# Rudrabha/Wav2Lip

Hardware: AMD Instinct MI355X
Metric: face-frames/sec (96x96, mel T=16) (higher is better)
Workload: dtype f32

## Files before the change

### include/w2l_hip.h

```cpp
#ifndef W2L_HIP_H
#define W2L_HIP_H

#include <stddef.h>
#include <stdint.h>

#ifdef __cplusplus
extern "C" {
#endif

#define W2L_OK 0
#define W2L_ERR_ARG (-1)
#define W2L_ERR_HIP (-2)
#define W2L_ERR_NOMEM (-3)

#define W2L_ACT_NONE 0
#define W2L_ACT_RELU 1
#define W2L_ACT_SIGMOID 2
#define W2L_ACT_LEAKY 3

#define W2L_PREC_F32 0
#define W2L_PREC_BF16 1

const char* w2l_last_error(void);
int w2l_abi_version(void);
// ... 201 lines not shown
                     float* dgamma, float* dbeta, float* dz, int dz_cs, float* g_out, int g_cs);
int w2l_act_bwd(void* stream, long long rows, int C, const float* dy, int dy_cs, const float* y, int y_cs, int act,
                const float* scale, float* dz, int dz_cs, float* g_out, int g_cs);
int w2l_add_rows(void* stream, long long rows, int C, const float* a, int a_cs, const float* b, int b_cs, float* out,
                 int out_cs);
int w2l_col_sum(void* stream, long long rows, int C, const float* x, int x_cs, float* out);

int w2l_l1_mean(void* stream, long long n, const float* a, const float* b, float* loss_out);
int w2l_l1_bwd(void* stream, long long n, const float* a, const float* b, const float* gout, float* da);
int w2l_cosine_bce_bwd(void* stream, int N, int C, const float* a, const float* v, const float* y, const float* gout,
                       float* da, float* dv);
int w2l_l2norm_bwd(void* stream, int N, int C, const float* x, int x_cs, const float* dy, float* dx, int dx_cs);
int w2l_bce_bwd(void* stream, int N, const float* p, const float* y, const float* gout, float* dp);

int w2l_shifted_pdist(void* stream, int T, int C, int vshift, const float* f1, const float* f2, float* out);

typedef struct w2l_adam_tensor {
    float* param;
    const float* grad;
    float* exp_avg;
    float* exp_avg_sq;
    long long n;
} w2l_adam_tensor;
typedef struct w2l_adam w2l_adam_t;
int w2l_adam_create(int ntensors, const long long* sizes_host, w2l_adam_t** out);
int w2l_adam_destroy(w2l_adam_t* h);
int w2l_adam_step(w2l_adam_t* h, void* stream, const w2l_adam_tensor* tensors_host, float lr, float beta1, float beta2,
                  float eps, float weight_decay, int step);


typedef struct w2l_plan w2l_plan_t;
int w2l_plan_create(w2l_plan_t** out);
int w2l_plan_destroy(w2l_plan_t* p);
int w2l_plan_add_conv(w2l_plan_t* p, const w2l_conv_t* c, int N, int H, int W, const float* x, int x_cs,
                      float* y, int y_cs, const float* res, int res_cs);
int w2l_plan_add_convb(w2l_plan_t* p, const w2l_convb_t* c, int N, int H, int W, const void* x, int x_cs, void* y, int y_cs,
                       const void* res, int res_cs, const float* scale, const float* shift);
int w2l_plan_add_convb_head(w2l_plan_t* p, const w2l_convb_t* c, int N, int H, int W, const void* x, int x_cs, uint8_t* frames,
                            float* y32, int y32_cs, const float* scale, const float* shift);
int w2l_plan_copy_item(w2l_plan_t* dst, const w2l_plan_t* src, int index);
int w2l_plan_run(const w2l_plan_t* p, void* stream);
int w2l_plan_size(const w2l_plan_t* p);
int w2l_plan_autotune(w2l_plan_t* p, void* stream, int reps);
int w2l_plan_get_config(const w2l_plan_t* p, int index, int* tile, int* ksplit);
int w2l_plan_set_config(w2l_plan_t* p, int index, int tile, int ksplit);
int w2l_plan_executed_flops(const w2l_plan_t* p, long long* flops_out, int* config_out);
int w2l_conv_num_igemm_tiles(void);
int w2l_flops_begin(void);
long long w2l_flops_end(long long* by_family);
int w2l_clock_probe(void* stream, int spin_us, unsigned long long* out2_dev);
int w2l_conv_config_family(int id);
int w2l_conv_exclude_families(int mask);
int w2l_igemm_block_order(int order, int order_r, int tiles_m, int tiles_n, int nphase, int* out);
int w2l_plan_profile(const w2l_plan_t* p, void* stream, int reps, float* ms_out);

#define W2L_TUNE_KEY_INTS 17
int w2l_tune_key_ints(void);
int w2l_tune_set(const int* key, int tile, int ksplit);
int w2l_tune_entry_applicable(const int* key, int tile);
int w2l_tune_clear(void);
int w2l_tune_count(void);
int w2l_tune_export(int* out, int cap_entries);

#ifdef __cplusplus
}
#endif
#endif
```

### wav2lip_amd/_lib.py

```python
import ctypes as C
import os

_HERE = os.path.dirname(os.path.abspath(__file__))
LIB_PATH = os.environ.get("W2L_HIP_LIB") or os.path.join(_HERE, "lib", "libw2l_hip.so")

ACT_NONE, ACT_RELU, ACT_SIGMOID, ACT_LEAKY = 0, 1, 2, 3
PREC_F32, PREC_BF16 = 0, 1


class ConvGeom(C.Structure):
    _fields_ = [(n, C.c_int) for n in
                ("transposed", "cin", "cout", "kh", "kw", "sh", "sw", "ph", "pw", "oph", "opw", "act")]


class AdamTensor(C.Structure):
    _fields_ = [("param", C.c_void_p), ("grad", C.c_void_p), ("exp_avg", C.c_void_p), ("exp_avg_sq", C.c_void_p),
                ("n", C.c_longlong)]


class WgradInfo(C.Structure):
    _fields_ = [(n, C.c_int) for n in ("family", "cfg", "ksplit", "chunk", "K", "kstep", "reduce_blocks")]


class WgradBf16Info(C.Structure):
# ... 82 lines not shown
                                     C.POINTER(C.c_int)]),
    "w2l_convb_forward_actbwd": (_i, [_vp, _vp, _i, _i, _i, _vp, _i, _vp, _i, _vp, _i, _vp, _i, _i, _vp, C.POINTER(C.c_int)]),
    "w2l_convb_set_tile": (_i, [_vp, _i]),
    "w2l_convb_num_tiles": (_i, []),
    "w2l_convb_resolve": (_i, [_vp, _i, _i, _i, _i, C.POINTER(C.c_int), C.POINTER(C.c_int), C.POINTER(C.c_int)]),
    "w2l_conv_wgrad_bf16": (_i, [C.POINTER(ConvGeom), _vp, _i, _i, _i, _vp, _i, _vp, _i, _vp]),
    "w2l_conv_wgrad_bf16_resolve": (_i, [C.POINTER(ConvGeom), _i, _i, _i, _i, _i, C.POINTER(WgradBf16Info)]),
    "w2l_bn_train_stats_bf16": (_i, [_vp, _ll, _i, _i, _vp, _i, _vp, _vp, _f, _f, _vp, _vp, _vp, _vp, _vp, _vp]),
    "w2l_affine_act_bf16": (_i, [_vp, _ll, _i, _vp, _i, _vp, _vp, _vp, _i, _i, _vp, _i]),
    "w2l_bn_train_bwd_bf16": (_i, [_vp, _ll, _i, _i, _vp, _i, _vp, _i, _vp, _i, _i, _vp, _vp, _vp, _vp, _vp, _vp, _vp, _i, _vp, _i]),
    "w2l_bn_train_bwd_apply_bf16": (_i, [_vp, _ll, _i, _vp, _i, _vp, _i, _vp, _i, _i, _vp, _vp, _vp, _vp, _vp, _vp, _vp, _i, _vp, _i]),
    "w2l_act_bwd_bf16": (_i, [_vp, _ll, _i, _vp, _i, _vp, _i, _i, _vp, _vp, _i, _vp, _i]),
    "w2l_add_rows_bf16": (_i, [_vp, _ll, _i, _vp, _i, _vp, _i, _vp, _i]),
    "w2l_col_sum_bf16": (_i, [_vp, _ll, _i, _vp, _i, _vp]),
    "w2l_thin1x1_forward_bf16": (_i, [_vp, _ll, _i, _i, _vp, _i, _vp, _vp, _i, _vp, _i]),
    "w2l_thin1x1_dgrad_bf16": (_i, [_vp, _ll, _i, _i, _vp, _i, _vp, _vp, _i, _vp, _i]),
    "w2l_thin1x1_wgrad_bf16": (_i, [_vp, _ll, _i, _i, _vp, _i, _vp, _i, _vp, _vp]),
    "w2l_thin1x1_wgrad_blocks": (_i, [_ll]),
    "w2l_nchw_to_nhwc_bf16": (_i, [_vp, _i, _i, _i, _i, _vp, _vp, _i, _i]),
    "w2l_nhwc_bf16_to_nchw": (_i, [_vp, _i, _i, _i, _i, _vp, _i, _vp]),
    "w2l_bn_train_stats": (_i, [_vp, _ll, _i, _vp, _i, _vp, _vp, _f, _f, _vp, _vp, _vp, _vp, _vp, _vp]),
    "w2l_affine_act": (_i, [_vp, _ll, _i, _vp, _i, _vp, _vp, _vp, _i, _i, _vp, _i]),
    "w2l_bn_train_bwd": (_i, [_vp, _ll, _i, _vp, _i, _vp, _i, _vp, _i, _i, _vp, _vp, _vp, _vp, _vp, _vp, _i, _vp, _i]),
    "w2l_act_bwd": (_i, [_vp, _ll, _i, _vp, _i, _vp, _i, _i, _vp, _vp, _i, _vp, _i]),
    "w2l_add_rows": (_i, [_vp, _ll, _i, _vp, _i, _vp, _i, _vp, _i]),
    "w2l_col_sum": (_i, [_vp, _ll, _i, _vp, _i, _vp]),
    "w2l_l1_mean": (_i, [_vp, _ll, _vp, _vp, _vp]),
    "w2l_l1_bwd": (_i, [_vp, _ll, _vp, _vp, _vp, _vp]),
    "w2l_cosine_bce_bwd": (_i, [_vp, _i, _i, _vp, _vp, _vp, _vp, _vp, _vp]),
    "w2l_l2norm_bwd": (_i, [_vp, _i, _i, _vp, _i, _vp, _vp, _i]),
    "w2l_bce_bwd": (_i, [_vp, _i, _vp, _vp, _vp, _vp]),
    "w2l_shifted_pdist": (_i, [_vp, _i, _i, _i, _vp, _vp, _vp]),
    "w2l_adam_create": (_i, [_i, C.POINTER(_ll), C.POINTER(_vp)]),
    "w2l_adam_destroy": (_i, [_vp]),
    "w2l_adam_step": (_i, [_vp, _vp, C.POINTER(AdamTensor), _f, _f, _f, _f, _f, _i]),
    "w2l_plan_create": (_i, [C.POINTER(_vp)]),
    "w2l_plan_destroy": (_i, [_vp]),
    "w2l_plan_add_conv": (_i, [_vp, _vp, _i, _i, _i, _vp, _i, _vp, _i, _vp, _i]),
    "w2l_plan_add_convb": (_i, [_vp, _vp, _i, _i, _i, _vp, _i, _vp, _i, _vp, _i, _vp, _vp]),
    "w2l_plan_add_convb_head": (_i, [_vp, _vp, _i, _i, _i, _vp, _i, _vp, _vp, _i, _vp, _vp]),
    "w2l_plan_copy_item": (_i, [_vp, _vp, _i]),
    "w2l_plan_run": (_i, [_vp, _vp]),
    "w2l_plan_size": (_i, [_vp]),
    "w2l_plan_autotune": (_i, [_vp, _vp, _i]),
    "w2l_plan_get_config": (_i, [_vp, _i, C.POINTER(_i), C.POINTER(_i)]),
    "w2l_plan_set_config": (_i, [_vp, _i, _i, _i]),
    "w2l_plan_profile": (_i, [_vp, _vp, _i, _vp]),
    "w2l_plan_executed_flops": (_i, [_vp, C.POINTER(_ll), C.POINTER(_i)]),
    "w2l_conv_num_igemm_tiles": (_i, []),
    "w2l_flops_begin": (_i, []),
    "w2l_flops_end": (_ll, [C.POINTER(_ll)]),
    "w2l_clock_probe": (C.c_int, [C.c_void_p, C.c_int, C.c_void_p]),
    "w2l_igemm_block_order": (C.c_int, [C.c_int, C.c_int, C.c_int, C.c_int, C.c_int, C.c_void_p]),
    "w2l_conv_config_family": (_i, [_i]),
    "w2l_conv_exclude_families": (_i, [_i]),
    "w2l_tune_key_ints": (_i, []),
    "w2l_tune_set": (_i, [C.POINTER(_i), _i, _i]),
    "w2l_tune_entry_applicable": (_i, [C.POINTER(_i), _i]),
    "w2l_tune_clear": (_i, []),
    "w2l_tune_count": (_i, []),
    "w2l_tune_export": (_i, [C.POINTER(_i), _i]),
}

_lib = None

TUNE_TABLE_PATH = os.path.join(_HERE, "tune_table.json")
EXACT = os.environ.get("W2L_EXACT", "0") == "1"
EXACT_TABLE_PATH = os.path.join(_HERE, "tune_table_exact.json")
FAMILY_NAMES = ("igemm", "wino", "wino2", "tp2", "wino4", "split", "wino2s", "tp2s", "stem7s", "k3s")
SPLIT_FAMILIES = frozenset(FAMILY_NAMES.index(n) for n in ("split", "wino2s", "tp2s", "stem7s", "k3s"))
FAMILY_WINO4, FAMILY_SPLIT, FAMILY_WINO2S, FAMILY_TP2S, FAMILY_STEM7S, FAMILY_K3S = (
    FAMILY_NAMES.index(n) for n in ("wino4", "split", "wino2s", "tp2s", "stem7s", "k3s"))


def config_ids(lib, family):
    f = FAMILY_NAMES.index(family)
    return [i for i in range(lib.w2l_conv_num_tiles()) if lib.w2l_conv_config_family(i) == f]


NO_SPLIT = os.environ.get("W2L_SPLIT", "1") == "0"
NOSPLIT_TABLE_PATH = os.path.join(_HERE, "tune_table_nosplit.json")


def load_tune_table(lib, path=None):
    import json
    if path is None and NO_SPLIT and not EXACT and not os.environ.get("W2L_TUNE_TABLE"):
        return load_tune_table(lib, TUNE_TABLE_PATH) + load_tune_table(lib, NOSPLIT_TABLE_PATH)
    path = path or os.environ.get("W2L_TUNE_TABLE") or (EXACT_TABLE_PATH if EXACT else TUNE_TABLE_PATH)
    if path == "0" or not os.path.exists(path):
        return 0
    with open(path) as fh:
        doc = json.load(fh)
    nk = lib.w2l_tune_key_ints()
    if doc.get("key_ints") != nk or doc.get("num_configs", 0) > lib.w2l_conv_num_tiles():
        raise RuntimeError("tune table %s was written for another library build (key_ints %s / configs %s)"
                           % (path, doc.get("key_ints"), doc.get("num_configs")))
    n = 0
    for e in doc["entries"]:
        key = (C.c_int * nk)(*e[:nk])
        check_rc = lib.w2l_tune_set(key, int(e[nk]), int(e[nk + 1]))
        if check_rc != 0:
            raise RuntimeError("tune table %s: bad entry %s" % (path, e))
        n += 1
    return n


# ... 58 lines not shown
```

### wav2lip_amd/csrc/conv_wino4.hip

```cpp
#include "w2l_common.h"
#include "w2l_pk.h"

namespace w2l {

typedef float f32x16 __attribute__((ext_vector_type(16)));
typedef unsigned int u32x4 __attribute__((ext_vector_type(4)));

__device__ __forceinline__ f32x2 pk2_mul4(f32x2 a) {
    f32x2 d;
    asm("v_pk_mul_f32 %0, %1, 4.0 op_sel_hi:[1,0]" : "=v"(d) : "v"(a));
    return d;
}

template <int BLK>
__device__ __forceinline__ void w4_at3(f32x2 m0, f32x2 m1, f32x2 m2, f32x2& o0, f32x2& o1, f32x2& o2, f32x2& o3) {
    if (BLK == 0) {
        const f32x2 sm = pk2_add(m1, m2);
        o1 = pk2_sub(m1, m2);
        o0 = pk2_add(m0, sm);
        o2 = sm;
        o3 = o1;
    } else {
        const f32x2 sm = pk2_add(m0, m1);
        const f32x2 df = pk2_sub(m0, m1);
// ... 9 lines not shown
    f32x2 R[4][3];
#pragma unroll
    for (int jl = 0; jl < 3; ++jl) {
        const f32x2 m0 = {acc[0 + jl][r], acc[0 + jl][r + 1]};
        const f32x2 m1 = {acc[3 + jl][r], acc[3 + jl][r + 1]};
        const f32x2 m2 = {acc[6 + jl][r], acc[6 + jl][r + 1]};
        w4_at3<PI>(m0, m1, m2, R[0][jl], R[1][jl], R[2][jl], R[3][jl]);
    }
    f32x2 P1[4];
#pragma unroll
    for (int oa = 0; oa < 4; ++oa) {
        f32x2 P[4];
        if (PI == 0 && oa == 3) {
#pragma unroll
            for (int ob = 0; ob < 4; ++ob) P[ob] = P1[ob];
        } else {
            w4_at3<PJ>(R[oa][0], R[oa][1], R[oa][2], P[0], P[1], P[2], P[3]);
        }
        if (oa == 1) {
#pragma unroll
            for (int ob = 0; ob < 4; ++ob) P1[ob] = P[ob];
        }
        float* yo = y + (oa * 4) * LDY;
#pragma unroll
        for (int ob = 0; ob < 4; ++ob) {
            yo[ob * LDY] = P[ob].x;
            yo[ob * LDY + tstride] = P[ob].y;
        }
    }
}

#ifndef W4_DBG
#define W4_DBG 0
#endif
#ifdef W4_TRACE
__device__ unsigned long long w4_trace_buf[256 * 16 * 8];
__device__ unsigned long long w4_trace_rt[256 * 16 * 2];
#define W4_STAMP(k)                                                                                              \
    do {                                                                                                         \
        if (threadIdx.x == 0 && trace_item < 16) {                                                               \
            w4_trace_buf[(blockIdx.x * 16 + trace_item) * 8 + (k)] = __builtin_readcyclecounter();              \
            if ((k) == 0 || (k) == 7)                                                                            \
                w4_trace_rt[(blockIdx.x * 16 + trace_item) * 2 + ((k) ? 1 : 0)] = __builtin_amdgcn_s_memrealtime(); \
        }                                                                                                        \
    } while (0)
#else
#define W4_STAMP(k)
#endif

constexpr unsigned kW4Oob = 0x80000000u;
constexpr int kW4BT = 32;
constexpr int kW4BC = 64;
constexpr int kW4KS = 8;
constexpr int kW4LDK = kW4KS + 4;
constexpr int kW4VPOS = kW4BT * kW4LDK;
constexpr int kW4VBUF = 36 * kW4VPOS;
constexpr int kW4NRAW = 3;
constexpr int kW4RAW4 = 512 * kW4NRAW;
constexpr int kW4PS = 186;
constexpr int kW4QS = 4 * kW4PS;
static_assert(2 * kW4QS <= kW4RAW4 && kW4PS % 8 == 2 && kW4QS % 16 == 8, "raw plane geometry");
constexpr int kW4LDY = kW4BC + 4;
constexpr int kW4LdsFloats = 2 * kW4VBUF + 2 * kW4RAW4 * 4;
constexpr int kW4LdsBytes = kW4LdsFloats * 4 + 2 * kW4BT * 4;
static_assert(4 * kW4BT * 4 * kW4LDY <= kW4LdsFloats, "one round of the four partial staging tiles must fit");
static_assert(kW4LdsBytes <= 160 * 1024, "LDS budget");

struct Wino4KArgs {
    const float* x;
    float* y;
    const float* res;
    const float* u;
    const float* scale;
    const float* shift;
    int N, H, W, cin, x_cs;
    int cout, y_cs, res_cs;
    int TH, TW;
    int bh, bw, ni;
    int nby, nbx, ngi;
    int RH, RW, R4;
    int pitch, istride;
    float inv_rw, inv_rh;
    int nks;
    int tiles_n;
    long long total;
    int act;
};

__global__ __launch_bounds__(512, 2) void conv_wino4_f32_kernel(const Wino4KArgs a) {
    extern __shared__ __attribute__((aligned(16))) char smem[];
    float* Vs = reinterpret_cast<float*>(smem);
    float* Rs = Vs + 2 * kW4VBUF;
    int* s_opix = reinterpret_cast<int*>(Rs + 2 * kW4RAW4 * 4);
    int* s_oflag = s_opix + kW4BT;

    const __amdgpu_buffer_rsrc_t rx = __builtin_amdgcn_make_buffer_rsrc(
        const_cast<float*>(a.x), 0, (int)((((long long)a.N * a.H * a.W - 1) * a.x_cs + a.cin) * 4), 0x00020000);

    const unsigned total = (unsigned)a.total;
    const unsigned per = (total + 7u) / 8u;
    const unsigned xcd = blockIdx.x & 7u, gw = gridDim.x >> 3;
#ifdef W4_TRACE
    int trace_item = -1;
#endif
    for (unsigned jw = blockIdx.x >> 3; jw < per; jw += gw) {
    const unsigned bid = xcd * per + jw;
    if (bid >= total) break;
#ifdef W4_TRACE
    ++trace_item;
#endif
    W4_STAMP(0);
    int t = threadIdx.x;
    asm volatile("" : "+v"(t));
    const int lane = t & 63;
    const int wave = __builtin_amdgcn_readfirstlane(t >> 6);
    const int wn = wave & 1;
    const int pb = wave >> 1;
    const int PI = pb >> 1, PJ = pb & 1;
    const int tile_n = (int)(bid % (unsigned)a.tiles_n);
    unsigned mb = bid / (unsigned)a.tiles_n;
    const int bx_i = (int)(mb % (unsigned)a.nbx);
    mb /= (unsigned)a.nbx;
    const int by_i = (int)(mb % (unsigned)a.nby);
    const int gi = (int)(mb / (unsigned)a.nby);
    const int n0 = tile_n * kW4BC;
    const int bhw = a.bh * a.bw;

    if (t < kW4BT) {
        const int il = t / bhw, r = t - il * bhw;
        const int tyl = r / a.bw, txl = r - tyl * a.bw;
        const int n = gi * a.ni + il, ty = by_i * a.bh + tyl, tx = bx_i * a.bw + txl;
        int o = -1, f = 0;
        if (il < a.ni && n < a.N && ty < a.TH && tx < a.TW) {
            o = (n * a.H + 4 * ty) * a.W + 4 * tx;
#pragma unroll
            for (int k = 0; k < 4; ++k) f |= ((4 * ty + k < a.H) ? (1 << k) : 0) | ((4 * tx + k < a.W) ? (16 << k) : 0);
        }
        s_opix[t] = o;
        s_oflag[t] = f;
    }

    unsigned goff[kW4NRAW];
    int rst[kW4NRAW];
#pragma unroll
    for (int k = 0; k < kW4NRAW; ++k) {
        const int e = t + 512 * k;
        const int q = (e >> 3) & 1, pix = (e >> 4) * 8 + (e & 7);
        unsigned off = kW4Oob;
        int st = -1;
        if (pix < a.R4) {
            const int p2 = (int)(((float)pix + 0.5f) * a.inv_rw);
            const int rxx = pix - p2 * a.RW;
            const int il = (int)(((float)p2 + 0.5f) * a.inv_rh);
            const int ry = p2 - il * a.RH;
            st = (q * kW4QS + (rxx & 3) * kW4PS + il * a.istride + ry * a.pitch + (rxx >> 2)) * 16;
            const int n = gi * a.ni + il;
            const int iy = 4 * by_i * a.bh - 1 + ry, ix = 4 * bx_i * a.bw - 1 + rxx;
            if (n < a.N && (unsigned)iy < (unsigned)a.H && (unsigned)ix < (unsigned)a.W)
                off = ((unsigned)((n * a.H + iy) * a.W + ix) * (unsigned)a.x_cs + (unsigned)(q * 4)) * 4u;
        }
        goff[k] = off;
        rst[k] = st;
    }
    f32x4 rawreg[kW4NRAW];
    auto raw_gload = [&](int step) {
        const unsigned soff = (unsigned)(step * kW4KS * 4);
#pragma unroll
        for (int k = 0; k < kW4NRAW; ++k)
            rawreg[k] = __builtin_bit_cast(f32x4, __builtin_amdgcn_raw_buffer_load_b128(rx, (int)goff[k], (int)soff, 0));
    };
    auto raw_store = [&](int buf) {
        char* dst = reinterpret_cast<char*>(Rs) + buf * (kW4RAW4 * 16);
#pragma unroll
        for (int k = 0; k < kW4NRAW; ++k)
            if (rst[k] >= 0) *reinterpret_cast<f32x4*>(dst + rst[k]) = rawreg[k];
    };

    const bool tf_wave = wave < 6;
    const int q = lane & 1;
    int ra, rb, rc, rd;
    float ca, cb, cc;
    switch (wave) {
        case 0: ra = 0; ca = 0.f; rb = 0; cb = 4.f; rc = 2; cc = -5.f; rd = 4; break;
        case 1: ra = 1; ca = -4.f; rb = 2; cb = -4.f; rc = 3; cc = 1.f; rd = 4; break;
        case 2: ra = 1; ca = 4.f; rb = 2; cb = -4.f; rc = 3; cc = -1.f; rd = 4; break;
        case 3: ra = 1; ca = -2.f; rb = 2; cb = -1.f; rc = 3; cc = 2.f; rd = 4; break;
        case 4: ra = 1; ca = 2.f; rb = 2; cb = -1.f; rc = 3; cc = -2.f; rd = 4; break;
        default: ra = 1; ca = 0.f; rb = 1; cb = 4.f; rc = 3; cc = -5.f; rd = 5; break;
    }
    int tf_base;
    {
        const int tl = lane >> 1;
        const int il = tl / bhw, r = tl - il * bhw;
        const int tyl = r / a.bw, txl = r - tyl * a.bw;
        const int ilc = il < a.ni ? il : 0;
        tf_base = (q * kW4QS + ilc * a.istride + 4 * tyl * a.pitch + txl) * 16;
    }
    const int rp = a.pitch * 16;
    const int o_a = tf_base + ra * rp, o_b = tf_base + rb * rp, o_c = tf_base + rc * rp, o_d = tf_base + rd * rp;
    float* const vwr = Vs + ((wave < 6 ? wave : 0) * 6) * kW4VPOS + (lane >> 1) * kW4LDK + q * 4;
    f32x4 rr[6];
    auto tf_rows = [&](int buf, int c0) {
        const char* src = reinterpret_cast<const char*>(Rs) + buf * (kW4RAW4 * 16);
#pragma unroll
        for (int c = c0; c < c0 + 1; ++c) {
            const int co = ((c & 3) * kW4PS + (c >> 2)) * 16;
            const f32x4 va = *reinterpret_cast<const f32x4*>(src + o_a + co), vb = *reinterpret_cast<const f32x4*>(src + o_b + co);
            const f32x4 vc = *reinterpret_cast<const f32x4*>(src + o_c + co), vd = *reinterpret_cast<const f32x4*>(src + o_d + co);
#pragma unroll
            for (int e = 0; e < 4; ++e) rr[c][e] = fmaf(ca, va[e], fmaf(cb, vb[e], fmaf(cc, vc[e], vd[e])));
        }
    };
    auto tf_cols_store = [&](int buf) {
        float* dst = vwr + buf * kW4VBUF;
        f32x4 v0, v1, v2, v3, v4, v5;
#pragma unroll
        for (int e = 0; e < 4; ++e) {
            const float p = fmaf(-4.f, rr[2][e], rr[4][e]);
            const float qq = fmaf(4.f, rr[1][e], -rr[3][e]);
            const float p2 = rr[4][e] - rr[2][e];
            const float q2 = 2.f * (rr[3][e] - rr[1][e]);
            v0[e] = fmaf(4.f, rr[0][e], fmaf(-5.f, rr[2][e], rr[4][e]));
            v1[e] = p - qq;
            v2[e] = p + qq;
            v3[e] = p2 + q2;
            v4[e] = p2 - q2;
            v5[e] = fmaf(4.f, rr[1][e], fmaf(-5.f, rr[3][e], rr[5][e]));
        }
        *reinterpret_cast<f32x4*>(dst + 0 * kW4VPOS) = v0;
        *reinterpret_cast<f32x4*>(dst + 1 * kW4VPOS) = v1;
        *reinterpret_cast<f32x4*>(dst + 2 * kW4VPOS) = v2;
        *reinterpret_cast<f32x4*>(dst + 3 * kW4VPOS) = v3;
        *reinterpret_cast<f32x4*>(dst + 4 * kW4VPOS) = v4;
        *reinterpret_cast<f32x4*>(dst + 5 * kW4VPOS) = v5;
    };

    const int nb = (n0 >> 5) + wn;
    const int F = a.nks * 36;
    const __amdgpu_buffer_rsrc_t ru = __builtin_amdgcn_make_buffer_rsrc(
        const_cast<float*>(a.u + (long long)nb * F * 256), 0, F * 1024, 0x00020000);
    const unsigned bl_lane = (unsigned)(lane * 16);
    const int pos0 = 18 * PI + 3 * PJ;
    const unsigned bl_pb = (unsigned)pos0 * 1024u;
    auto bload = [&](int kc, int s) {
        const unsigned soff = (unsigned)kc * 36864u + bl_pb + (unsigned)(6 * (s / 3) + (s % 3)) * 1024u;
        return __builtin_bit_cast(f32x4, __builtin_amdgcn_raw_buffer_load_b128(ru, (int)bl_lane, (int)soff, 0));
    };
    constexpr int RING = 3;
    f32x4 bq[RING];

    f32x16 acc[9];
#pragma unroll
    for (int s = 0; s < 9; ++s)
#pragma unroll
        for (int r = 0; r < 16; ++r) acc[s][r] = 0.f;

    const int nsteps = a.cin / kW4KS;
    raw_gload(0);
#pragma unroll
    for (int i = 0; i < RING; ++i) bq[i] = bload(0, i);
    raw_store(0);
    raw_gload(1);
    __syncthreads();
    W4_STAMP(1);
    if (tf_wave) {
#pragma unroll
        for (int c = 0; c < 6; ++c) tf_rows(0, c);
        tf_cols_store(0);
    }
    raw_store(1);
    __syncthreads();
    W4_STAMP(2);

    const float* Abase = Vs + pos0 * kW4VPOS + (lane & 31) * kW4LDK + (lane >> 5) * 4;
    for (int step = 0; step < nsteps; ++step) {
        const int buf = step & 1;
        const float* Ab = Abase + buf * kW4VBUF;
        f32x4 af = *reinterpret_cast<const f32x4*>(Ab);
#pragma unroll
        for (int s = 0; s < 9; ++s) {
            const f32x4 ac = af;
            if (s < 8) af = *reinterpret_cast<const f32x4*>(Ab + (6 * ((s + 1) / 3) + ((s + 1) % 3)) * kW4VPOS);
            const f32x4 bc = bq[s % RING];
#if !(W4_DBG & 8)
            bq[s % RING] = (s < 9 - RING) ? bload(step, s + RING) : bload(step + 1, s + RING - 9);
#endif
            if (s == 0) {
                if (!(W4_DBG & 4)) raw_gload(step + 2);
            } else if (s >= 1 && s <= 6) {
                if (!(W4_DBG & 2) && tf_wave) tf_rows(buf ^ 1, s - 1);
            } else if (s == 7) {
                if (!(W4_DBG & 2) && tf_wave) tf_cols_store(buf ^ 1);
            } else if (s == 8) {
                if (!(W4_DBG & 4)) raw_store(buf);
            }
            __builtin_amdgcn_sched_barrier(0);
#if W4_DBG & 1
            asm volatile("" : "+v"(acc[s]) : "v"(ac), "v"(bc));
#else
#pragma unroll
            for (int e = 0; e < 4; ++e) acc[s] = __builtin_amdgcn_mfma_f32_32x32x2f32(ac[e], bc[e], acc[s], 0, 0, 0);
#endif
            __builtin_amdgcn_sched_barrier(0);
        }
        __syncthreads();
    }

    W4_STAMP(3);
    float* Ys = Vs;
    const long long npix = (long long)a.N * a.H * a.W;
    const __amdgpu_buffer_rsrc_t ry =
        __builtin_amdgcn_make_buffer_rsrc(a.y, 0, (int)(((npix - 1) * a.y_cs + a.cout) * 4), 0x00020000);
    const __amdgpu_buffer_rsrc_t rres = __builtin_amdgcn_make_buffer_rsrc(
        const_cast<float*>(a.res ? a.res : a.y), 0, a.res ? (int)(((npix - 1) * a.res_cs + a.cout) * 4) : 0, 0x00020000);
    constexpr int CG = kW4BC / 4;
    const int c4 = t % CG;
    const int ch = n0 + c4 * 4;
    const f32x4 sc = *reinterpret_cast<const f32x4*>(a.scale + ch);
    const f32x4 sh = *reinterpret_cast<const f32x4*>(a.shift + ch);
    const float neg_slope = a.act == W2L_ACT_RELU ? 0.f : (a.act == W2L_ACT_LEAKY ? 0.01f : 1.f);
    constexpr int kPart = 8 * 16 * kW4LDY;
    constexpr int NIT = 8 * 16 * CG / 512;
    auto out_pix = [&](int round, int i) {
        const int id = i * 512 + t;
        const int pxl = id / CG;
        const int tile = 8 * round + (pxl >> 4), oa = (pxl >> 2) & 3, ob = pxl & 3;
        const int opix = s_opix[tile];
        const int fl = s_oflag[tile];
        const bool ok = (opix >= 0) & (((fl >> oa) & 1) != 0) & (((fl >> (4 + ob)) & 1) != 0);
        return ok ? opix + oa * a.W + ob : -1;
    };
    f32x4 rv[NIT];
    auto res_load = [&](int round) {
#pragma unroll
        for (int i = 0; i < NIT; ++i) {
            const int pix = out_pix(round, i);
            rv[i] = __builtin_bit_cast(f32x4, __builtin_amdgcn_raw_buffer_load_b128(
                rres, (int)(pix >= 0 ? ((unsigned)pix * (unsigned)a.res_cs + (unsigned)ch) * 4u : kW4Oob), 0, 0));
        }
    };
    res_load(0);
#pragma unroll
    for (int round = 0; round < 4; ++round) {
        {
            float* yrow = Ys + pb * kPart + wn * 32 + (lane & 31) + (4 * (lane >> 5)) * 16 * kW4LDY;
            constexpr int TS = 16 * kW4LDY;
            if (pb == 0) {
                w4_partial_store<0, 0, kW4LDY>(acc, 4 * round, yrow, TS);
                w4_partial_store<0, 0, kW4LDY>(acc, 4 * round + 2, yrow + 2 * TS, TS);
            } else if (pb == 1) {
                w4_partial_store<0, 1, kW4LDY>(acc, 4 * round, yrow, TS);
                w4_partial_store<0, 1, kW4LDY>(acc, 4 * round + 2, yrow + 2 * TS, TS);
            } else if (pb == 2) {
                w4_partial_store<1, 0, kW4LDY>(acc, 4 * round, yrow, TS);
                w4_partial_store<1, 0, kW4LDY>(acc, 4 * round + 2, yrow + 2 * TS, TS);
            } else {
                w4_partial_store<1, 1, kW4LDY>(acc, 4 * round, yrow, TS);
                w4_partial_store<1, 1, kW4LDY>(acc, 4 * round + 2, yrow + 2 * TS, TS);
            }
        }
        __syncthreads();
#pragma unroll
        for (int i = 0; i < NIT; ++i) {
            const int id = i * 512 + t;
            const int pix = out_pix(round, i);
            const bool ok = pix >= 0;
            const f32x4 rvv = rv[i];
            const float* src = Ys + (id / CG) * kW4LDY + c4 * 4;
            const f32x4 p0 = *reinterpret_cast<const f32x4*>(src);
            const f32x4 p1 = *reinterpret_cast<const f32x4*>(src + kPart);
            const f32x4 p2 = *reinterpret_cast<const f32x4*>(src + 2 * kPart);
            const f32x4 p3 = *reinterpret_cast<const f32x4*>(src + 3 * kPart);
            f32x4 v;
#pragma unroll
            for (int e = 0; e < 4; ++e) {
                const float xv = fmaf((p0[e] + p1[e]) + (p2[e] + p3[e]), sc[e], sh[e]) + rvv[e];
                v[e] = fmaf(neg_slope, fminf(xv, 0.f), fmaxf(xv, 0.f));
            }
            __builtin_amdgcn_raw_buffer_store_b128(
                __builtin_bit_cast(u32x4, v), ry, (int)(ok ? ((unsigned)pix * (unsigned)a.y_cs + (unsigned)ch) * 4u : kW4Oob), 0, 0);
        }
        if (round < 3) res_load(round + 1);
        __syncthreads();
        W4_STAMP(4 + round);
    }
    }
}

struct Wino4PackArgs {
    const float* w;
    float* u;
    int cin, cout;
    int transposed;
};

__global__ void wino4_pack_kernel(const Wino4PackArgs a) {
    const int total = a.cout * a.cin;
    const int nks = a.cin / 8;
    constexpr double G[6][3] = {{0.25, 0.0, 0.0},          {-1.0 / 6, -1.0 / 6, -1.0 / 6}, {-1.0 / 6, 1.0 / 6, -1.0 / 6},
                                {1.0 / 24, 1.0 / 12, 1.0 / 6}, {1.0 / 24, -1.0 / 12, 1.0 / 6}, {0.0, 0.0, 1.0}};
    for (int j = blockIdx.x * blockDim.x + threadIdx.x; j < total; j += gridDim.x * blockDim.x) {
        const int e = j & 3, n = (j >> 2) & 31, h = (j >> 7) & 1;
        const int blk = j >> 8;
        const int kc = blk % nks, nbk = blk / nks;
        const int co = nbk * 32 + n;
        const int ci = kc * 8 + 4 * h + e;
        const float* g = a.transposed ? a.w + ((long long)ci * a.cout + co) * 9 : a.w + ((long long)co * a.cin + ci) * 9;
        double gd[3][3];
#pragma unroll
        for (int aa = 0; aa < 3; ++aa)
#pragma unroll
            for (int bb = 0; bb < 3; ++bb) gd[aa][bb] = (double)(a.transposed ? g[(2 - aa) * 3 + (2 - bb)] : g[aa * 3 + bb]);
        float* dst = a.u + (long long)blk * 36 * 256 + (j & 255);
#pragma unroll
        for (int pi = 0; pi < 6; ++pi)
#pragma unroll
            for (int pj = 0; pj < 6; ++pj) {
                double sum = 0.0;
#pragma unroll
                for (int aa = 0; aa < 3; ++aa)
#pragma unroll
                    for (int bb = 0; bb < 3; ++bb) sum += G[pi][aa] * gd[aa][bb] * G[pj][bb];
                dst[(pi * 6 + pj) * 256] = (float)sum;
            }
    }
}

struct W4Block { int bh, bw, ni; };
static const W4Block kW4Blocks[] = {{4, 8, 1}, {8, 4, 1}, {4, 4, 2}, {2, 8, 2}, {8, 2, 1}, {2, 4, 3}, {4, 2, 3}, {3, 3, 3},
                                    {2, 2, 6}, {2, 3, 4}, {3, 2, 4}, {1, 4, 6}, {4, 1, 5}, {1, 2, 10}, {2, 1, 9}, {1, 1, 15}};

static bool wino4_block_fits(const W4Block& b) {
    const int RH = 4 * b.bh + 2, RW = 4 * b.bw + 2;
    return b.bh * b.bw * b.ni <= kW4BT && b.ni * RH * RW * 2 <= kW4RAW4 && b.ni * RH * (b.bw + 1) <= kW4PS;
}

static void wino4_plane_geom(const W4Block& b, int* pitch, int* istride) {
    static const int kGroup[2][16] = {{0, 1, 2, 3, 12, 13, 14, 15, 20, 21, 22, 23, 24, 25, 26, 27},
                                      {4, 5, 6, 7, 8, 9, 10, 11, 16, 17, 18, 19, 28, 29, 30, 31}};
    const int RH = 4 * b.bh + 2, bhw = b.bh * b.bw;
    int best = 1 << 30;
    *pitch = b.bw + 1;
    *istride = RH * (b.bw + 1);
    for (int p = b.bw + 1; p <= b.bw + 4; ++p)
        for (int is = RH * p; is <= RH * p + 15; ++is) {
            if (b.ni * is > kW4PS) break;
            int cost = (p - b.bw - 1) + (is - RH * p);
            for (int g = 0; g < 4; ++g) {
                int cnt[16] = {0};
                for (int k = 0; k < 16; ++k) {
                    const int lane = kGroup[g & 1][k] + 32 * (g >> 1);
                    const int tl = lane >> 1, q = lane & 1;
                    const int il = tl / bhw, r = tl % bhw;
                    const int ilc = il < b.ni ? il : 0;
                    ++cnt[(q * kW4QS + ilc * is + 4 * (r / b.bw) * p + r % b.bw) & 15];
                }
                for (int k = 0; k < 16; ++k) cost += cnt[k] > 1 ? (cnt[k] - 1) * 64 * cnt[k] : 0;
            }
            if (cost < best) { best = cost; *pitch = p; *istride = is; }
        }
}

static W4Block wino4_pick_block(int N, int TH, int TW) {
    W4Block best = {1, 1, 1};
    double best_cost = 1e300;
    for (const W4Block& b : kW4Blocks) {
        if (!wino4_block_fits(b)) continue;
        const double items = (double)ceil_div(TH, b.bh) * ceil_div(TW, b.bw) * ceil_div(N, b.ni);
        const double halo = (double)(4 * b.bh + 2) * (4 * b.bw + 2) / (16.0 * b.bh * b.bw);
        const double cost = items * (1.0 + 0.05 * halo);
        if (cost < best_cost) { best_cost = cost; best = b; }
    }
    return best;
}

bool wino4_ok(int cin, int cout) { return cin % kW4KS == 0 && cout % kW4BC == 0; }

long long wino4_u_floats(int cin, int cout) { return (long long)cout * cin * 36; }

int wino4_pack(const float* w, float* u, int cin, int cout, int transposed, hipStream_t stream) {
    Wino4PackArgs pa;
    pa.w = w; pa.u = u; pa.cin = cin; pa.cout = cout; pa.transposed = transposed;
    long long blocks = ((long long)cin * cout + 255) / 256;
    if (blocks > 8192) blocks = 8192;
    hipLaunchKernelGGL(wino4_pack_kernel, dim3((unsigned)blocks), dim3(256), 0, stream, pa);
    W2L_HIP_CHECK(hipGetLastError());
    return W2L_OK;
}

int wino4_init_attrs() {
    static bool done = false;
    if (done) return W2L_OK;
    W2L_HIP_CHECK(hipFuncSetAttribute(reinterpret_cast<const void*>(conv_wino4_f32_kernel),
                                      hipFuncAttributeMaxDynamicSharedMemorySize, kW4LdsBytes));
    done = true;
    return W2L_OK;
}

int wino4_launch(const WinoKArgs& w, const float* u4, hipStream_t stream, long long* flops_out) {
    Wino4KArgs a;
    a.x = w.x; a.y = w.y; a.res = w.res; a.u = u4; a.scale = w.scale; a.shift = w.shift;
    a.N = w.N; a.H = w.H; a.W = w.W; a.cin = w.cin; a.x_cs = w.x_cs;
    a.cout = w.cout; a.y_cs = w.y_cs; a.res_cs = w.res_cs; a.act = w.act;
    a.TH = (a.H + 3) / 4;
    a.TW = (a.W + 3) / 4;
    const W4Block b = wino4_pick_block(a.N, a.TH, a.TW);
    a.bh = b.bh; a.bw = b.bw; a.ni = b.ni;
    a.nby = ceil_div(a.TH, b.bh);
    a.nbx = ceil_div(a.TW, b.bw);
    a.ngi = ceil_div(a.N, b.ni);
    a.RH = 4 * b.bh + 2;
    a.RW = 4 * b.bw + 2;
    a.R4 = b.ni * a.RH * a.RW;
    wino4_plane_geom(b, &a.pitch, &a.istride);
    a.inv_rw = 1.0f / (float)a.RW;
    a.inv_rh = 1.0f / (float)a.RH;
    a.nks = a.cin / 8;
    a.tiles_n = a.cout / kW4BC;
    a.total = (long long)a.ngi * a.nby * a.nbx * a.tiles_n;
    W2L_REQUIRE(a.total < (1ll << 31), "grid too large");
    W2L_REQUIRE((long long)a.N * a.H * a.W < (1ll << 31), "tensor too large");
    if (flops_out) {
        *flops_out = 2ll * 36 * a.total * kW4BT * kW4BC * a.cin;
        return W2L_OK;
    }
    long long grid = (a.total + 7) / 8 * 8;
    if (grid > 256) grid = 256;
    hipLaunchKernelGGL(conv_wino4_f32_kernel, dim3((unsigned)grid), dim3(512), kW4LdsBytes, stream, a);
    W2L_HIP_CHECK(hipGetLastError());
    return W2L_OK;
}

}

#ifdef W4_TRACE
extern "C" int w2l_dbg_w4_trace(unsigned long long* out) {
    if (hipMemcpyFromSymbol(out, HIP_SYMBOL(w2l::w4_trace_buf), sizeof(w2l::w4_trace_buf)) != hipSuccess) return 1;
    return (int)hipMemcpyFromSymbol(out + 256 * 16 * 8, HIP_SYMBOL(w2l::w4_trace_rt), sizeof(w2l::w4_trace_rt));
}
#endif
```

Measured before the change: 29000.

## Split wino4 tail tiles into half-width items and swizzle unpadded LDS layout

Reworks the Winograd F(4,3) kernel's work distribution so that when the last wave of tiles would leave most CUs idle, the leftover tiles are split into two 32-channel halves to balance the tail. It also removes the LDS row padding in favour of an XOR swizzle, enlarges the raw input plane, and adds an NRAW=4 variant plus a larger 2x2x8 block shape. The aim is better CU utilisation on the final round and more block choices, at the cost of half-width items that leave half the waves idle during the MFMA loop. A host-side item-order query is added for inspection.

```diff
diff --git a/include/w2l_hip.h b/include/w2l_hip.h
--- a/include/w2l_hip.h
+++ b/include/w2l_hip.h
@@ -277,6 +277,7 @@
 int w2l_conv_config_family(int id);
 int w2l_conv_exclude_families(int mask);
 int w2l_igemm_block_order(int order, int order_r, int tiles_m, int tiles_n, int nphase, int* out);
+int w2l_wino4_item_order(int N, int H, int W, int cout, int* info, int* out);
 int w2l_plan_profile(const w2l_plan_t* p, void* stream, int reps, float* ms_out);
 
 #define W2L_TUNE_KEY_INTS 17
diff --git a/wav2lip_amd/_lib.py b/wav2lip_amd/_lib.py
--- a/wav2lip_amd/_lib.py
+++ b/wav2lip_amd/_lib.py
@@ -158,6 +158,7 @@
     "w2l_flops_end": (_ll, [C.POINTER(_ll)]),
     "w2l_clock_probe": (C.c_int, [C.c_void_p, C.c_int, C.c_void_p]),
     "w2l_igemm_block_order": (C.c_int, [C.c_int, C.c_int, C.c_int, C.c_int, C.c_int, C.c_void_p]),
+    "w2l_wino4_item_order": (_i, [_i, _i, _i, _i, C.c_void_p, C.c_void_p]),
     "w2l_conv_config_family": (_i, [_i]),
     "w2l_conv_exclude_families": (_i, [_i]),
     "w2l_tune_key_ints": (_i, []),
diff --git a/wav2lip_amd/csrc/conv_wino4.hip b/wav2lip_amd/csrc/conv_wino4.hip
--- a/wav2lip_amd/csrc/conv_wino4.hip
+++ b/wav2lip_amd/csrc/conv_wino4.hip
@@ -85,19 +85,20 @@
 constexpr int kW4BT = 32;
 constexpr int kW4BC = 64;
 constexpr int kW4KS = 8;
-constexpr int kW4LDK = kW4KS + 4;
+constexpr int kW4LDK = kW4KS;
 constexpr int kW4VPOS = kW4BT * kW4LDK;
 constexpr int kW4VBUF = 36 * kW4VPOS;
-constexpr int kW4NRAW = 3;
-constexpr int kW4RAW4 = 512 * kW4NRAW;
-constexpr int kW4PS = 186;
+constexpr int kW4MaxRaw = 4;
+constexpr int kW4PS = 250;
 constexpr int kW4QS = 4 * kW4PS;
-static_assert(2 * kW4QS <= kW4RAW4 && kW4PS % 8 == 2 && kW4QS % 16 == 8, "raw plane geometry");
+constexpr int kW4RAW4 = 2 * kW4QS;
+static_assert(kW4PS % 8 == 2 && kW4QS % 16 == 8, "raw plane geometry");
 constexpr int kW4LDY = kW4BC + 4;
-constexpr int kW4LdsFloats = 2 * kW4VBUF + 2 * kW4RAW4 * 4;
+constexpr int kW4KFloats = 2 * kW4VBUF + 2 * kW4RAW4 * 4;
+constexpr int kW4YFloats = 4 * kW4BT * 4 * kW4LDY;
+constexpr int kW4LdsFloats = kW4KFloats > kW4YFloats ? kW4KFloats : kW4YFloats;
 constexpr int kW4LdsBytes = kW4LdsFloats * 4 + 2 * kW4BT * 4;
-static_assert(4 * kW4BT * 4 * kW4LDY <= kW4LdsFloats, "one round of the four partial staging tiles must fit");
-static_assert(kW4LdsBytes <= 160 * 1024, "LDS budget");
+static_assert(kW4LdsBytes <= 159744 + 256, "LDS stays at or below what the padded layout took");
 
 struct Wino4KArgs {
     const float* x;
@@ -116,47 +117,47 @@
     float inv_rw, inv_rh;
     int nks;
     int tiles_n;
-    long long total;
+    unsigned nfull;
+    unsigned nhalf;
     int act;
 };
 
-__global__ __launch_bounds__(512, 2) void conv_wino4_f32_kernel(const Wino4KArgs a) {
-    extern __shared__ __attribute__((aligned(16))) char smem[];
-    float* Vs = reinterpret_cast<float*>(smem);
-    float* Rs = Vs + 2 * kW4VBUF;
-    int* s_opix = reinterpret_cast<int*>(Rs + 2 * kW4RAW4 * 4);
-    int* s_oflag = s_opix + kW4BT;
-
-    const __amdgpu_buffer_rsrc_t rx = __builtin_amdgcn_make_buffer_rsrc(
-        const_cast<float*>(a.x), 0, (int)((((long long)a.N * a.H * a.W - 1) * a.x_cs + a.cin) * 4), 0x00020000);
-
-    const unsigned total = (unsigned)a.total;
-    const unsigned per = (total + 7u) / 8u;
-    const unsigned xcd = blockIdx.x & 7u, gw = gridDim.x >> 3;
-#ifdef W4_TRACE
-    int trace_item = -1;
-#endif
-    for (unsigned jw = blockIdx.x >> 3; jw < per; jw += gw) {
-    const unsigned bid = xcd * per + jw;
-    if (bid >= total) break;
-#ifdef W4_TRACE
-    ++trace_item;
-#endif
+__host__ __device__ __forceinline__ int w4_item_decode(unsigned xcd, unsigned jw, unsigned nfull, unsigned nhalf, unsigned tiles_n,
+                                                       unsigned* mb, int* n0) {
+    const unsigned per_full = (nfull + 7u) >> 3;
+    if (jw < per_full) {
+        const unsigned bid = xcd * per_full + jw;
+        if (bid >= nfull) return 0;
+        *mb = bid / tiles_n;
+        *n0 = (int)(bid % tiles_n) * kW4BC;
+        return 64;
+    }
+    const unsigned hid = xcd * ((nhalf + 7u) >> 3) + (jw - per_full);
+    if (hid >= nhalf) return 0;
+    const unsigned bid = nfull + (hid >> 1);
+    *mb = bid / tiles_n;
+    *n0 = (int)(bid % tiles_n) * kW4BC + (int)(hid & 1u) * 32;
+    return 32;
+}
+__host__ __device__ __forceinline__ unsigned w4_list_len(unsigned nfull, unsigned nhalf) { return ((nfull + 7u) >> 3) + ((nhalf + 7u) >> 3); }
+
+template <int BC, int NRAW>
+__device__ __forceinline__ void w4_item(const Wino4KArgs& a, float* Vs, float* Rs, int* s_opix, int* s_oflag,
+                                        const __amdgpu_buffer_rsrc_t rx, unsigned mb, const int n0, const int trace_item) {
+    static_assert((BC == 64 || BC == 32) && NRAW <= kW4MaxRaw, "item form");
     W4_STAMP(0);
     int t = threadIdx.x;
     asm volatile("" : "+v"(t));
     const int lane = t & 63;
     const int wave = __builtin_amdgcn_readfirstlane(t >> 6);
-    const int wn = wave & 1;
-    const int pb = wave >> 1;
+    const bool mm = BC == 64 || wave < 4;
+    const int wn = BC == 64 ? (wave & 1) : 0;
+    const int pb = BC == 64 ? (wave >> 1) : (wave & 3);
     const int PI = pb >> 1, PJ = pb & 1;
-    const int tile_n = (int)(bid % (unsigned)a.tiles_n);
-    unsigned mb = bid / (unsigned)a.tiles_n;
     const int bx_i = (int)(mb % (unsigned)a.nbx);
     mb /= (unsigned)a.nbx;
     const int by_i = (int)(mb % (unsigned)a.nby);
     const int gi = (int)(mb / (unsigned)a.nby);
-    const int n0 = tile_n * kW4BC;
     const int bhw = a.bh * a.bw;
 
     if (t < kW4BT) {
@@ -173,10 +174,10 @@
         s_oflag[t] = f;
     }
 
-    unsigned goff[kW4NRAW];
-    int rst[kW4NRAW];
-#pragma unroll
-    for (int k = 0; k < kW4NRAW; ++k) {
+    unsigned goff[NRAW];
+    int rst[NRAW];
+#pragma unroll
+    for (int k = 0; k < NRAW; ++k) {
         const int e = t + 512 * k;
         const int q = (e >> 3) & 1, pix = (e >> 4) * 8 + (e & 7);
         unsigned off = kW4Oob;
@@ -195,17 +196,17 @@
         goff[k] = off;
         rst[k] = st;
     }
-    f32x4 rawreg[kW4NRAW];
+    f32x4 rawreg[NRAW];
     auto raw_gload = [&](int step) {
         const unsigned soff = (unsigned)(step * kW4KS * 4);
 #pragma unroll
-        for (int k = 0; k < kW4NRAW; ++k)
+        for (int k = 0; k < NRAW; ++k)
             rawreg[k] = __builtin_bit_cast(f32x4, __builtin_amdgcn_raw_buffer_load_b128(rx, (int)goff[k], (int)soff, 0));
     };
     auto raw_store = [&](int buf) {
         char* dst = reinterpret_cast<char*>(Rs) + buf * (kW4RAW4 * 16);
 #pragma unroll
-        for (int k = 0; k < kW4NRAW; ++k)
+        for (int k = 0; k < NRAW; ++k)
             if (rst[k] >= 0) *reinterpret_cast<f32x4*>(dst + rst[k]) = rawreg[k];
     };
 
@@ -231,7 +232,7 @@
     }
     const int rp = a.pitch * 16;
     const int o_a = tf_base + ra * rp, o_b = tf_base + rb * rp, o_c = tf_base + rc * rp, o_d = tf_base + rd * rp;
-    float* const vwr = Vs + ((wave < 6 ? wave : 0) * 6) * kW4VPOS + (lane >> 1) * kW4LDK + q * 4;
+    float* const vwr = Vs + ((wave < 6 ? wave : 0) * 6) * kW4VPOS + (lane >> 1) * kW4LDK + (q ^ ((lane >> 4) & 1)) * 4;
     f32x4 rr[6];
     auto tf_rows = [&](int buf, int c0) {
         const char* src = reinterpret_cast<const char*>(Rs) + buf * (kW4RAW4 * 16);
@@ -280,7 +281,7 @@
         return __builtin_bit_cast(f32x4, __builtin_amdgcn_raw_buffer_load_b128(ru, (int)bl_lane, (int)soff, 0));
     };
     constexpr int RING = 3;
-    f32x4 bq[RING];
+    f32x4 bq[RING] = {};
 
     f32x16 acc[9];
 #pragma unroll
@@ -290,8 +291,10 @@
 
     const int nsteps = a.cin / kW4KS;
     raw_gload(0);
-#pragma unroll
-    for (int i = 0; i < RING; ++i) bq[i] = bload(0, i);
+    if (mm) {
+#pragma unroll
+        for (int i = 0; i < RING; ++i) bq[i] = bload(0, i);
+    }
     raw_store(0);
     raw_gload(1);
     __syncthreads();
@@ -305,19 +308,22 @@
     __syncthreads();
     W4_STAMP(2);
 
-    const float* Abase = Vs + pos0 * kW4VPOS + (lane & 31) * kW4LDK + (lane >> 5) * 4;
+    const float* Abase = Vs + pos0 * kW4VPOS + (lane & 31) * kW4LDK + ((lane >> 5) ^ ((lane >> 3) & 1)) * 4;
     for (int step = 0; step < nsteps; ++step) {
         const int buf = step & 1;
         const float* Ab = Abase + buf * kW4VBUF;
-        f32x4 af = *reinterpret_cast<const f32x4*>(Ab);
+        f32x4 af = {};
+        if (mm) af = *reinterpret_cast<const f32x4*>(Ab);
 #pragma unroll
         for (int s = 0; s < 9; ++s) {
             const f32x4 ac = af;
-            if (s < 8) af = *reinterpret_cast<const f32x4*>(Ab + (6 * ((s + 1) / 3) + ((s + 1) % 3)) * kW4VPOS);
             const f32x4 bc = bq[s % RING];
+            if (mm) {
+                if (s < 8) af = *reinterpret_cast<const f32x4*>(Ab + (6 * ((s + 1) / 3) + ((s + 1) % 3)) * kW4VPOS);
 #if !(W4_DBG & 8)
-            bq[s % RING] = (s < 9 - RING) ? bload(step, s + RING) : bload(step + 1, s + RING - 9);
+                bq[s % RING] = (s < 9 - RING) ? bload(step, s + RING) : bload(step + 1, s + RING - 9);
 #endif
+            }
             if (s == 0) {
                 if (!(W4_DBG & 4)) raw_gload(step + 2);
             } else if (s >= 1 && s <= 6) {
@@ -331,8 +337,10 @@
 #if W4_DBG & 1
             asm volatile("" : "+v"(acc[s]) : "v"(ac), "v"(bc));
 #else
-#pragma unroll
-            for (int e = 0; e < 4; ++e) acc[s] = __builtin_amdgcn_mfma_f32_32x32x2f32(ac[e], bc[e], acc[s], 0, 0, 0);
+            if (mm) {
+#pragma unroll
+                for (int e = 0; e < 4; ++e) acc[s] = __builtin_amdgcn_mfma_f32_32x32x2f32(ac[e], bc[e], acc[s], 0, 0, 0);
+            }
 #endif
             __builtin_amdgcn_sched_barrier(0);
         }
@@ -346,14 +354,16 @@
         __builtin_amdgcn_make_buffer_rsrc(a.y, 0, (int)(((npix - 1) * a.y_cs + a.cout) * 4), 0x00020000);
     const __amdgpu_buffer_rsrc_t rres = __builtin_amdgcn_make_buffer_rsrc(
         const_cast<float*>(a.res ? a.res : a.y), 0, a.res ? (int)(((npix - 1) * a.res_cs + a.cout) * 4) : 0, 0x00020000);
-    constexpr int CG = kW4BC / 4;
+    constexpr int LDY = BC + 4;
+    constexpr int CG = BC / 4;
     const int c4 = t % CG;
     const int ch = n0 + c4 * 4;
     const f32x4 sc = *reinterpret_cast<const f32x4*>(a.scale + ch);
     const f32x4 sh = *reinterpret_cast<const f32x4*>(a.shift + ch);
     const float neg_slope = a.act == W2L_ACT_RELU ? 0.f : (a.act == W2L_ACT_LEAKY ? 0.01f : 1.f);
-    constexpr int kPart = 8 * 16 * kW4LDY;
+    constexpr int kPart = 8 * 16 * LDY;
     constexpr int NIT = 8 * 16 * CG / 512;
+    static_assert(4 * kPart <= kW4LdsFloats, "one round of the four partial staging tiles must fit");
     auto out_pix = [&](int round, int i) {
         const int id = i * 512 + t;
         const int pxl = id / CG;
@@ -375,21 +385,21 @@
     res_load(0);
 #pragma unroll
     for (int round = 0; round < 4; ++round) {
-        {
-            float* yrow = Ys + pb * kPart + wn * 32 + (lane & 31) + (4 * (lane >> 5)) * 16 * kW4LDY;
-            constexpr int TS = 16 * kW4LDY;
+        if (mm) {
+            float* yrow = Ys + pb * kPart + wn * 32 + (lane & 31) + (4 * (lane >> 5)) * 16 * LDY;
+            constexpr int TS = 16 * LDY;
             if (pb == 0) {
-                w4_partial_store<0, 0, kW4LDY>(acc, 4 * round, yrow, TS);
-                w4_partial_store<0, 0, kW4LDY>(acc, 4 * round + 2, yrow + 2 * TS, TS);
+                w4_partial_store<0, 0, LDY>(acc, 4 * round, yrow, TS);
+                w4_partial_store<0, 0, LDY>(acc, 4 * round + 2, yrow + 2 * TS, TS);
             } else if (pb == 1) {
-                w4_partial_store<0, 1, kW4LDY>(acc, 4 * round, yrow, TS);
-                w4_partial_store<0, 1, kW4LDY>(acc, 4 * round + 2, yrow + 2 * TS, TS);
+                w4_partial_store<0, 1, LDY>(acc, 4 * round, yrow, TS);
+                w4_partial_store<0, 1, LDY>(acc, 4 * round + 2, yrow + 2 * TS, TS);
             } else if (pb == 2) {
-                w4_partial_store<1, 0, kW4LDY>(acc, 4 * round, yrow, TS);
-                w4_partial_store<1, 0, kW4LDY>(acc, 4 * round + 2, yrow + 2 * TS, TS);
+                w4_partial_store<1, 0, LDY>(acc, 4 * round, yrow, TS);
+                w4_partial_store<1, 0, LDY>(acc, 4 * round + 2, yrow + 2 * TS, TS);
             } else {
-                w4_partial_store<1, 1, kW4LDY>(acc, 4 * round, yrow, TS);
-                w4_partial_store<1, 1, kW4LDY>(acc, 4 * round + 2, yrow + 2 * TS, TS);
+                w4_partial_store<1, 1, LDY>(acc, 4 * round, yrow, TS);
+                w4_partial_store<1, 1, LDY>(acc, 4 * round + 2, yrow + 2 * TS, TS);
             }
         }
         __syncthreads();
@@ -399,7 +409,7 @@
             const int pix = out_pix(round, i);
             const bool ok = pix >= 0;
             const f32x4 rvv = rv[i];
-            const float* src = Ys + (id / CG) * kW4LDY + c4 * 4;
+            const float* src = Ys + (id / CG) * LDY + c4 * 4;
             const f32x4 p0 = *reinterpret_cast<const f32x4*>(src);
             const f32x4 p1 = *reinterpret_cast<const f32x4*>(src + kPart);
             const f32x4 p2 = *reinterpret_cast<const f32x4*>(src + 2 * kPart);
@@ -417,6 +427,32 @@
         __syncthreads();
         W4_STAMP(4 + round);
     }
+}
+
+template <int NRAW>
+__global__ __launch_bounds__(512, 2) void conv_wino4_f32_kernel(const Wino4KArgs a) {
+    extern __shared__ __attribute__((aligned(16))) char smem[];
+    float* Vs = reinterpret_cast<float*>(smem);
+    float* Rs = Vs + 2 * kW4VBUF;
+    int* s_opix = reinterpret_cast<int*>(Vs + kW4LdsFloats);
+    int* s_oflag = s_opix + kW4BT;
+
+    const __amdgpu_buffer_rsrc_t rx = __builtin_amdgcn_make_buffer_rsrc(
+        const_cast<float*>(a.x), 0, (int)((((long long)a.N * a.H * a.W - 1) * a.x_cs + a.cin) * 4), 0x00020000);
+
+    const unsigned len = w4_list_len(a.nfull, a.nhalf);
+    const unsigned xcd = blockIdx.x & 7u, gw = gridDim.x >> 3;
+    int trace_item = -1;
+    for (unsigned jw = blockIdx.x >> 3; jw < len; jw += gw) {
+        unsigned mb = 0;
+        int n0 = 0;
+        const int bc = w4_item_decode(xcd, jw, a.nfull, a.nhalf, (unsigned)a.tiles_n, &mb, &n0);
+        if (bc == 0) continue;
+        ++trace_item;
+        if (bc == 64)
+            w4_item<64, NRAW>(a, Vs, Rs, s_opix, s_oflag, rx, mb, n0, trace_item);
+        else
+            w4_item<32, NRAW>(a, Vs, Rs, s_opix, s_oflag, rx, mb, n0, trace_item);
     }
 }
 
@@ -460,12 +496,12 @@
 }
 
 struct W4Block { int bh, bw, ni; };
-static const W4Block kW4Blocks[] = {{4, 8, 1}, {8, 4, 1}, {4, 4, 2}, {2, 8, 2}, {8, 2, 1}, {2, 4, 3}, {4, 2, 3}, {3, 3, 3},
+static const W4Block kW4Blocks[] = {{4, 8, 1}, {8, 4, 1}, {4, 4, 2}, {2, 8, 2}, {8, 2, 1}, {2, 4, 3}, {4, 2, 3}, {3, 3, 3}, {2, 2, 8},
                                     {2, 2, 6}, {2, 3, 4}, {3, 2, 4}, {1, 4, 6}, {4, 1, 5}, {1, 2, 10}, {2, 1, 9}, {1, 1, 15}};
 
 static bool wino4_block_fits(const W4Block& b) {
     const int RH = 4 * b.bh + 2, RW = 4 * b.bw + 2;
-    return b.bh * b.bw * b.ni <= kW4BT && b.ni * RH * RW * 2 <= kW4RAW4 && b.ni * RH * (b.bw + 1) <= kW4PS;
+    return b.bh * b.bw * b.ni <= kW4BT && b.ni * RH * RW * 2 <= 512 * kW4MaxRaw && b.ni * RH * (b.bw + 1) <= kW4PS;
 }
 
 static void wino4_plane_geom(const W4Block& b, int* pitch, int* istride) {
@@ -524,17 +560,17 @@
 int wino4_init_attrs() {
     static bool done = false;
     if (done) return W2L_OK;
-    W2L_HIP_CHECK(hipFuncSetAttribute(reinterpret_cast<const void*>(conv_wino4_f32_kernel),
+    W2L_HIP_CHECK(hipFuncSetAttribute(reinterpret_cast<const void*>(conv_wino4_f32_kernel<3>),
+                                      hipFuncAttributeMaxDynamicSharedMemorySize, kW4LdsBytes));
+    W2L_HIP_CHECK(hipFuncSetAttribute(reinterpret_cast<const void*>(conv_wino4_f32_kernel<4>),
                                       hipFuncAttributeMaxDynamicSharedMemorySize, kW4LdsBytes));
     done = true;
     return W2L_OK;
 }
 
-int wino4_launch(const WinoKArgs& w, const float* u4, hipStream_t stream, long long* flops_out) {
-    Wino4KArgs a;
-    a.x = w.x; a.y = w.y; a.res = w.res; a.u = u4; a.scale = w.scale; a.shift = w.shift;
-    a.N = w.N; a.H = w.H; a.W = w.W; a.cin = w.cin; a.x_cs = w.x_cs;
-    a.cout = w.cout; a.y_cs = w.y_cs; a.res_cs = w.res_cs; a.act = w.act;
+constexpr unsigned kW4CUs = 256;
+
+static int wino4_plan(Wino4KArgs& a, unsigned* grid) {
     a.TH = (a.H + 3) / 4;
     a.TW = (a.W + 3) / 4;
     const W4Block b = wino4_pick_block(a.N, a.TH, a.TW);
@@ -550,20 +586,66 @@
     a.inv_rh = 1.0f / (float)a.RH;
     a.nks = a.cin / 8;
     a.tiles_n = a.cout / kW4BC;
-    a.total = (long long)a.ngi * a.nby * a.nbx * a.tiles_n;
-    W2L_REQUIRE(a.total < (1ll << 31), "grid too large");
+    const long long total = (long long)a.ngi * a.nby * a.nbx * a.tiles_n;
+    W2L_REQUIRE(total < (1ll << 30), "grid too large");
     W2L_REQUIRE((long long)a.N * a.H * a.W < (1ll << 31), "tensor too large");
+    const unsigned left = (unsigned)(total % kW4CUs);
+    const bool split = left > 0 && 2 * left <= kW4CUs;
+    a.nfull = (unsigned)total - (split ? left : 0u);
+    a.nhalf = split ? 2 * left : 0u;
+    const unsigned entries = a.nfull + a.nhalf;
+    *grid = entries >= kW4CUs ? kW4CUs : (entries + 7u) / 8u * 8u;
+    return W2L_OK;
+}
+
+int wino4_launch(const WinoKArgs& w, const float* u4, hipStream_t stream, long long* flops_out) {
+    Wino4KArgs a;
+    a.x = w.x; a.y = w.y; a.res = w.res; a.u = u4; a.scale = w.scale; a.shift = w.shift;
+    a.N = w.N; a.H = w.H; a.W = w.W; a.cin = w.cin; a.x_cs = w.x_cs;
+    a.cout = w.cout; a.y_cs = w.y_cs; a.res_cs = w.res_cs; a.act = w.act;
+    unsigned grid = 0;
+    if (const int rc = wino4_plan(a, &grid)) return rc;
     if (flops_out) {
-        *flops_out = 2ll * 36 * a.total * kW4BT * kW4BC * a.cin;
+        *flops_out = 2ll * 36 * ((long long)a.nfull + a.nhalf / 2) * kW4BT * kW4BC * a.cin;
         return W2L_OK;
     }
-    long long grid = (a.total + 7) / 8 * 8;
-    if (grid > 256) grid = 256;
-    hipLaunchKernelGGL(conv_wino4_f32_kernel, dim3((unsigned)grid), dim3(512), kW4LdsBytes, stream, a);
+    if (2 * a.R4 <= 512 * 3)
+        hipLaunchKernelGGL(conv_wino4_f32_kernel<3>, dim3(grid), dim3(512), kW4LdsBytes, stream, a);
+    else
+        hipLaunchKernelGGL(conv_wino4_f32_kernel<4>, dim3(grid), dim3(512), kW4LdsBytes, stream, a);
     W2L_HIP_CHECK(hipGetLastError());
     return W2L_OK;
 }
 
+}
+
+extern "C" int w2l_wino4_item_order(int N, int H, int W, int cout, int* info, int* out) {
+    using namespace w2l;
+    W2L_REQUIRE(info && N >= 1 && H >= 1 && W >= 1 && cout >= kW4BC && cout % kW4BC == 0, "wino4_item_order: bad arguments");
+    Wino4KArgs a = {};
+    a.N = N; a.H = H; a.W = W; a.cin = kW4KS; a.cout = cout;
+    unsigned grid = 0;
+    if (const int rc = wino4_plan(a, &grid)) return rc;
+    const int v[12] = {a.bh, a.bw, a.ni, (int)(a.nfull + a.nhalf / 2), (int)a.nfull, (int)a.nhalf, (int)grid, kW4LdsBytes,
+                       2 * a.R4 <= 512 * 3 ? 3 : 4, a.pitch, a.istride, kW4PS};
+    for (int i = 0; i < 12; ++i) info[i] = v[i];
+    if (!out) return W2L_OK;
+    const unsigned len = w4_list_len(a.nfull, a.nhalf), gw = grid >> 3;
+    for (unsigned blk = 0; blk < grid; ++blk)
+        for (unsigned jw = blk >> 3; jw < len; jw += gw) {
+            unsigned mb = 0;
+            int n0 = 0;
+            const int bc = w4_item_decode(blk & 7u, jw, a.nfull, a.nhalf, (unsigned)a.tiles_n, &mb, &n0);
+            if (bc == 0) continue;
+            out[0] = (int)blk;
+            out[1] = (int)(mb / ((unsigned)a.nbx * a.nby));
+            out[2] = (int)(mb / (unsigned)a.nbx % (unsigned)a.nby);
+            out[3] = (int)(mb % (unsigned)a.nbx);
+            out[4] = n0;
+            out[5] = bc;
+            out += 6;
+        }
+    return W2L_OK;
 }
 
 #ifdef W4_TRACE
```

After: 29190, median of 6. Within noise of the previous version (+0.7%).
